# 0xC0000054/pdn-jpegxl

Hardware: AMD Instinct MI355X
Metric: megapixels/sec decode (4K lossy VarDCT) (higher is better)
Workload: dtype f32

## Files before the change

### pdn_jpegxl_amd/csrc/decoder.cc

```cpp
#include <hip/hip_runtime.h>
#include <algorithm>
#include <atomic>
#include <cmath>
#include <cstdarg>
#include <cstdio>
#include <cstdlib>
#include <cstring>
#include <memory>
#include <mutex>
#include <string>
#include <thread>
#include <vector>
#include "../../include/jxlfiletypeio.h"
#include "entropy_plan.h"
#include "host_parse.h"
#include "icc.h"
#include "kernels.h"

namespace jxlhip {

struct HipError : std::runtime_error {
  explicit HipError(const std::string& m) : std::runtime_error(m) {}
};
#define HIP_OK(expr)                                                                                      \
// ... 78 lines not shown
  hipStream_t own_stream = nullptr;
  float* d_basis_all = nullptr;
  float* d_basis_small = nullptr;
  float* d_basis_mfma = nullptr;
  float* d_llf_scale = nullptr;
  uint16_t* d_natural[kNumOrders] = {};
  U32x2* d_scan[kNumQuantTables] = {};
  float* d_dq[kNumQuantTables] = {};
  uint32_t dq_n[kNumQuantTables] = {};
  struct Tap { std::vector<uint8_t> qcoef[3], xyb_idct[3], xyb_filtered[3], noise_rnd[3], noise[3]; };
  struct Slot {
    uint8_t* d_ws = nullptr; size_t ws_cap = 0;
    uint8_t* d_blob = nullptr; size_t blob_cap = 0;
    uint8_t* h_blob = nullptr; size_t h_blob_cap = 0;
    uint32_t* h_status = nullptr; size_t h_status_cap = 0;
    int n = 0;
    std::vector<ParsedFrame> frames;
    int nfiles = 0;
    std::vector<int> file_of;
    std::vector<ParsedFrame> files;
    std::vector<DevImage> imgs;
    std::vector<int> parse_status;
    std::vector<std::string> parse_msg;
    std::vector<size_t> status_off;
    DevImage* d_imgs = nullptr;
    bool pending = false;
    hipEvent_t lf_done = nullptr, hf_done = nullptr, done = nullptr, uploaded = nullptr;
    std::vector<Tap> taps;
    std::vector<std::string> stage_names;
    std::vector<int> stage_chain;
    std::vector<hipEvent_t> events;
    std::vector<float> stage_ms;
  };
  static constexpr int kSlots = 3;
  static constexpr int kPixelChunk = 32;
  Slot slots[kSlots];
  int cur = 0, last = 0;
  Slot* active = &slots[0];
  hipStream_t stream_lf = nullptr;
  hipStream_t stream_hf = nullptr;
  hipStream_t last_stream = nullptr;
  std::vector<std::string> total_names;
  std::vector<double> total_ms;
  int total_batches = 0;
  std::string sticky_error;
  int sticky_status = 0;
  uint8_t* li_dev = nullptr; uint8_t* li_host = nullptr; size_t li_cap = 0;
  void EnsureLoadImageBuffers(size_t bytes);
  int lane_stride_override = 0;
  int hf_stride_override = 0;
  bool debug_taps = false;
  int band_first_row = 0, band_rows = 0;
  bool no_stream_pairs = false;
  bool no_lf_pipeline = false;
  bool no_direct = false, mod_lanes64 = false;
  bool overlap = true;
  int downscale = 1;

  explicit JxlHipDecoder(int dev);
  ~JxlHipDecoder();
  void EnsureWs(size_t bytes);
  void EnsureBlob(size_t bytes);
  void Mark(const char* name, hipStream_t s, int chain);
  void WaitSlot(Slot& S);
  Slot& Last() { return slots[last]; }
  void Decode(int32_t n_, const uint8_t* const* host_data, const size_t* sizes, const uint8_t* const* dev_data,
              uint8_t* const* dev_out, hipStream_t stream, bool sync, DecoderStatus* statuses, ErrorInfo* err);
  DecoderStatus Finish(DecoderStatus* statuses, ErrorInfo* err);
  void CopyPlaneTap(int stage);
  void PrepassSingle(ParsedFrame& f, const uint8_t* dev_file);
  EntropyPlanOptions PlanOptions() const;
};

JxlHipDecoder::JxlHipDecoder(int dev) {
  if (dev < 0) HIP_OK(hipGetDevice(&dev));
  device = dev;
  HIP_OK(hipSetDevice(device));
  int entropy_cus = 0, pixel_cus = 0;
  if (const char* e = Knob("JXLHIP_ENTROPY_CUS")) entropy_cus = std::min(256, std::max(0, atoi(e)));
  if (const char* e = Knob("JXLHIP_PIXEL_CUS")) pixel_cus = std::min(256, std::max(0, atoi(e)));
  auto masked_stream = [](hipStream_t* s, int first, int count) {
    uint32_t mask[8] = {0, 0, 0, 0, 0, 0, 0, 0};
    for (int i = first; i < first + count; i++) mask[i >> 5] |= 1u << (i & 31);
    HIP_OK(hipExtStreamCreateWithCUMask(s, 8, mask));
  };
  if (pixel_cus) masked_stream(&own_stream, 256 - pixel_cus, pixel_cus);
  else HIP_OK(hipStreamCreateWithFlags(&own_stream, hipStreamNonBlocking));
  int prio_least = 0, prio_greatest = 0;
  (void)hipDeviceGetStreamPriorityRange(&prio_least, &prio_greatest);
  const int prio = Knob("JXLHIP_NO_PRIORITY") ? prio_least : prio_greatest;
  if (entropy_cus) {
    masked_stream(&stream_lf, 0, entropy_cus);
    masked_stream(&stream_hf, 0, entropy_cus);
  } else {
    HIP_OK(hipStreamCreateWithPriority(&stream_lf, hipStreamNonBlocking, prio));
    HIP_OK(hipStreamCreateWithPriority(&stream_hf, hipStreamNonBlocking, prio));
  }
  for (auto& S : slots) {
    HIP_OK(hipEventCreateWithFlags(&S.lf_done, hipEventDisableTiming));
    HIP_OK(hipEventCreateWithFlags(&S.hf_done, hipEventDisableTiming));
    HIP_OK(hipEventCreateWithFlags(&S.done, hipEventDisableTiming));
    HIP_OK(hipEventCreateWithFlags(&S.uploaded, hipEventDisableTiming));
  }
  if (const char* e = Knob("JXLHIP_NO_OVERLAP")) overlap = atoi(e) == 0;
  const StaticTables& st = GetStaticTables();
  std::vector<float> all;
// ... 978 lines not shown
  if (s_lf != s_hf) {
    HIP_OK(hipEventRecord(S.lf_done, s_lf));
    HIP_OK(hipStreamWaitEvent(s_hf, S.lf_done, 0));
  }
#ifdef JXLHIP_EXPERIMENTS
  if (const char* e = Knob("JXLHIP_INTERFERE")) {
    int kind = 0, wgs = 1, lds_kb = 64; float ms = 100.f;
    if (sscanf(e, "%d,%d,%d,%f", &kind, &wgs, &lds_kb, &ms) >= 1 && kind >= 1 && kind <= 6 && wgs >= 1 && wgs <= 16 && lds_kb >= 1 && lds_kb <= 160 && ms > 0 && ms < 2000) {
      static hipStream_t xs = nullptr;
      static float* xbuf = nullptr;
      const size_t xbytes = (size_t)512 << 20;
      if (!xs) { HIP_OK(hipStreamCreateWithFlags(&xs, hipStreamNonBlocking)); HIP_OK(hipMalloc(&xbuf, xbytes)); }
      if (s_lf != s_hf) HIP_OK(hipStreamWaitEvent(xs, S.lf_done, 0));
      LaunchInterference(kind, wgs, lds_kb, ms, xbuf, xbytes, xs);
    }
  }
#endif
  Mark("hf_start", s_hf, 1);
  if (!(skip_stages & 2) && (!ds || npass_t))
  LaunchHfDecode(d_imgs, (const SectionTask*)(d_blob + off_pass_tasks), npass_t, plan.hf_waves * 64, plan.lane_stride, plan.hf.Bytes(), plan.lds_hf_lanes, s_hf);
  if (!ds || npass_t) Mark("hf_decode", s_hf, 1);
  if (any_alpha && !(skip_stages & 4))
    LaunchAlphaAns(d_imgs, (const SectionTask*)(d_blob + off_alpha_tasks), nalpha_t, plan.alpha_stride, plan.alpha.Bytes(), plan.direct_alpha, plan.lean_mod, s_hf);
  if (!ds || any_alpha) Mark("alpha_ans", s_hf, 1);
  if (debug_taps && !ds) {
    taps.assign(n, Tap());
    LaunchExpandCoefficients(d_imgs, n, true, max_tiles, stream);
    HIP_OK(hipStreamSynchronize(stream));
    CopyPlaneTap(0);
  }
  const bool finish_on_hf = s_hf == stream || debug_taps || !Knob("JXLHIP_ALPHA_FINISH_ON_PIX");
  if (finish_on_hf) {
    if (any_alpha && !(skip_stages & 4)) LaunchAlphaFinish(d_imgs, n, max_groups, s_hf);
    if (!ds || any_alpha) Mark("alpha_finish", s_hf, 1);
  }
  if (s_hf != stream) {
    HIP_OK(hipEventRecord(S.hf_done, s_hf));
    HIP_OK(hipStreamWaitEvent(stream, S.hf_done, 0));
  }
  Mark("main_start", stream, 2);
  if (!finish_on_hf) {
    if (any_alpha && !(skip_stages & 4)) LaunchAlphaFinish(d_imgs, n, max_groups, stream);
    Mark("alpha_finish", stream, 2);
  }
  hipStream_t s_pix = pix_on_hf ? s_hf : stream;
  if (ds && any_vardct) {
    if (any_alpha) LaunchAlphaReduce(d_imgs, n, max_ds_cells, s_pix);
    LaunchLfOutput(d_imgs, n, max_ds_cells, s_pix);
    Mark("lf_output", s_pix, 2);
  }
  for (int c0 = 0; c0 < (ds ? 0 : n); c0 += pixel_chunk) {
    const int cnt = std::min(pixel_chunk, n - c0);
    if (!(skip_stages & 8))
    LaunchReconTiles(d_imgs + c0, cnt, max_tiles, d_basis_all, d_basis_small, d_llf_scale, d_basis_mfma, s_pix);
    Mark("reconstruct", s_pix, 2);
    LaunchExpandCoefficients(d_imgs + c0, cnt, false, max_tiles, s_pix);
    LaunchGenericReconstruct(d_imgs + c0, cnt, d_basis_all, d_basis_small, d_llf_scale, s_pix);
    Mark("reconstruct_generic", s_pix, 2);
    if (debug_taps) { HIP_OK(hipStreamSynchronize(s_pix)); CopyPlaneTap(1); }
    if (any_noise && !(early_noise && c0 == 0)) { LaunchNoise(d_imgs + c0, cnt, max_groups, max_w, max_h, s_pix); Mark("noise", s_pix, 2); }
    if (!(skip_stages & 16))
    LaunchFilterTiles(d_imgs + c0, cnt, max_w, max_h, stage_mask, any_unfiltered, any_fused, any_fused2, s_pix);
    Mark("filters+output", s_pix, 2);
  }
  if (s_pix != stream) {
    HIP_OK(hipEventRecord(S.hf_done, s_pix));
    HIP_OK(hipStreamWaitEvent(stream, S.hf_done, 0));
  }
  if (nmod_t) {
    if (s_lf != stream) { HIP_OK(hipEventRecord(S.lf_done, s_lf)); HIP_OK(hipStreamWaitEvent(stream, S.lf_done, 0)); }
    LaunchModularAns(d_imgs, n, (const SectionTask*)(d_blob + off_mod_tasks), nmod_t, plan.mod.Bytes(), plan.max_mod_groups,
                     plan.max_mod_coded, plan.mod_lanes, plan.mod_rb, plan.mod_wp_lds, plan.direct_mod, stream);
    for (auto& op : mod_ops) {
      if (op.kind == 3) LaunchModularPalette(op.a, op.b, op.out, op.nout, op.type, op.rw, op.rh, op.status, stream);
      else LaunchModularOp(op.kind, op.a, op.b, op.c, op.aw, op.ah, op.rw, op.rh, op.type, stream);
    }
    LaunchModularOut(d_imgs, n, max_mod_pixels, stream);
    if (ds) LaunchBoxReduce(d_imgs, n, max_ds_cells, stream);
    Mark("modular", stream, 2);
  }
  if (!patch_tiles.empty()) {
    LaunchPatches((const PatchFrame*)(d_blob + off_patch_frames), (const PatchTile*)(d_blob + off_patch_tiles), (int)patch_tiles.size(),
                  (const int32_t*)(d_blob + off_patch_list), (const PatchPos*)(d_blob + off_patch_pos), (const PatchRef*)(d_blob + off_patch_refs),
                  stream);
    Mark("patches", stream, 2);
  }
  if (!comps.empty()) {
    LaunchCompose((const ComposeImage*)(d_blob + off_comp_imgs), (const ComposeFrame*)(d_blob + off_comp_frames), (int)comps.size(), max_segments, stream);
    Mark("compose", stream, 2);
  }
  for (int i = 0; i < n; i++)
    if (parse_status[i] == DecoderStatus_Ok && frames[i].orientation != 1 && !ds) {
      const ParsedFrame& f = frames[i];
      LaunchOrient(imgs[i].out, dev_out[i], (int)f.xsize, (int)f.ysize, (f.ncolor + (f.black_index >= 0 ? 1 : 0) + (f.alpha_index >= 0 ? 1 : 0)) * (int)OutBytesPerSample(f),
                   (int)f.orientation, stream);
    }
  LaunchStatusToHost((const uint32_t*)(d_ws + z_status_base), h_status, n * 16, stream);
  HIP_OK(hipEventRecord(S.done, stream));
  HIP_OK(hipGetLastError());
  last_stream = stream;
  S.pending = true;
  last = cur;
  cur = (cur + 1) % kSlots;
  (void)max_padded;
  if (sync) {
    DecoderStatus st = Finish(statuses, err);
    (void)st;
// ... 205 lines not shown
    info->num_channels = f.ncolor + (f.black_index >= 0 ? 1 : 0) + info->has_alpha;
    info->bytes_per_sample = (int32_t)OutBytesPerSample(f);
    info->reserved = f.exp_bits ? 1 : 0;
    info->xsize_blocks = f.w8; info->ysize_blocks = f.h8;
    info->num_groups = f.ng; info->num_lf_groups = f.nlf;
    info->epf_iters = f.epf_iters; info->gaborish = f.gab;
    info->codestream_bytes = f.cs_size;
    return DecoderStatus_Ok;
  } catch (const ParseError& e) {
    SetErr(err, "%s", e.what());
    return e.status;
  } catch (const std::exception& e) {
    SetErr(err, "%s", e.what());
    return DecoderStatus_DecodeError;
  }
}

DecoderStatus jxlhip_decode_batch(JxlHipDecoder* dec, int32_t n, const uint8_t* const* host_data, const size_t* sizes,
                                  const uint8_t* const* dev_data, uint8_t* const* dev_out, void* stream, int32_t synchronize,
                                  DecoderStatus* statuses, ErrorInfo* err) {
  if (!dec || !host_data || !sizes || !dev_out || n <= 0) return DecoderStatus_NullParameter;
  try {
    dec->Decode(n, host_data, sizes, dev_data, dev_out, (hipStream_t)stream, synchronize != 0, statuses, err);
    if (statuses) for (int i = 0; i < n; i++) if (statuses[i] != DecoderStatus_Ok) return statuses[i];
    return DecoderStatus_Ok;
  } catch (const std::bad_alloc&) {
    return DecoderStatus_OutOfMemory;
  } catch (const std::exception& e) {
    SetErr(err, "%s", e.what());
    return DecoderStatus_DecodeError;
  }
}

DecoderStatus jxlhip_finish(JxlHipDecoder* dec, DecoderStatus* statuses, ErrorInfo* err) {
  if (!dec) return DecoderStatus_NullParameter;
  try {
    return dec->Finish(statuses, err);
  } catch (const std::exception& e) {
    SetErr(err, "%s", e.what());
    return DecoderStatus_DecodeError;
  }
}

int32_t jxlhip_set_option(JxlHipDecoder* dec, const char* name, int32_t value) {
  if (!dec || !name) return 0;
  if (!strcmp(name, "debug_taps")) { dec->debug_taps = value != 0; return 1; }
  if (!strcmp(name, "query_pixel_chunk")) return JxlHipDecoder::kPixelChunk;
  if (!strcmp(name, "lane_stride")) { if (value != 0 && !PowerOfTwoUpTo64(value)) return 0; dec->lane_stride_override = value; return 1; }
  if (!strcmp(name, "band_first_row")) { if (value < 0) return 0; dec->band_first_row = value; return 1; }
  if (!strcmp(name, "band_rows")) { if (value < 0) return 0; dec->band_rows = value; return 1; }
  if (!strcmp(name, "no_direct")) { dec->no_direct = value != 0; return 1; }
  if (!strcmp(name, "no_stream_pairs")) { dec->no_stream_pairs = value != 0; return 1; }
  if (!strcmp(name, "no_lf_pipeline")) { dec->no_lf_pipeline = value != 0; return 1; }
  if (!strcmp(name, "mod_lanes64")) { dec->mod_lanes64 = value != 0; return 1; }
  if (!strcmp(name, "overlap")) { dec->overlap = value != 0; return 1; }
  if (!strcmp(name, "downscale")) { if (value != 1 && value != 8) return 0; dec->downscale = value; return 1; }
  return 0;
}

size_t jxlhip_read_plane(JxlHipDecoder* dec, int32_t index, const char* name, int32_t channel, void* dst, size_t capacity) {
  if (!dec || !name) return 0;
  JxlHipDecoder::Slot& S = dec->Last();
  if (index < 0 || index >= S.n || S.pending) return 0;
  if (S.parse_status[index] != DecoderStatus_Ok) return 0;
  const DevImage& d = S.imgs[index];
  std::string nm(name);
  const size_t cells = (size_t)d.w8 * d.h8, pix = (size_t)d.wp * d.hp;
  const void* src = nullptr;
  size_t bytes = 0;
  bool host = false;
  const int c = std::min(2, std::max(0, channel));
  if (nm == "lf") { src = d.lf_final[c]; bytes = cells * 4; }
  else if (nm == "lf_quant") { src = d.lfq[c]; bytes = cells * 4; }
  else if (nm == "cellinfo") { src = d.cellinfo; bytes = cells * 4; }
  else if (nm == "raw_quant") { src = d.rawq; bytes = cells * 2; }
  else if (nm == "sharpness") { src = d.sharp; bytes = cells; }
  else if (nm == "ytox") { src = d.ytox; bytes = (size_t)d.wt * d.ht; }
  else if (nm == "ytob") { src = d.ytob; bytes = (size_t)d.wt * d.ht; }
  else if (nm == "alpha") { src = d.alpha; bytes = (size_t)d.w * d.h; }
  else if (nm == "inv_sigma") { src = d.inv_sigma; bytes = cells * 4; }
  else if (dec->debug_taps && (size_t)index < S.taps.size()) {
    host = true;
    if (nm == "qcoef") { src = S.taps[index].qcoef[c].data(); bytes = S.taps[index].qcoef[c].size(); }
    else if (nm == "xyb_idct") { src = S.taps[index].xyb_idct[c].data(); bytes = S.taps[index].xyb_idct[c].size(); }
    else if (nm == "xyb_filtered") { src = S.taps[index].xyb_filtered[c].data(); bytes = S.taps[index].xyb_filtered[c].size(); }
    else if (nm == "noise_rnd") { src = S.taps[index].noise_rnd[c].data(); bytes = S.taps[index].noise_rnd[c].size(); }
    else if (nm == "noise") { src = S.taps[index].noise[c].data(); bytes = S.taps[index].noise[c].size(); }
  }
  (void)pix;
  if (!src || !bytes) return 0;
  if (dst && capacity) {
    size_t nb = std::min(bytes, capacity);
    if (host) memcpy(dst, src, nb);
    else if (hipMemcpy(dst, src, nb, hipMemcpyDeviceToHost) != hipSuccess) return 0;
  }
  return bytes;
}

int32_t jxlhip_stage_times(JxlHipDecoder* dec, const char** names, float* ms, int32_t capacity) {
  if (!dec) return 0;
  JxlHipDecoder::Slot& S = dec->Last();
  int32_t k = 0;
  for (size_t i = 1; i < S.stage_names.size() && i < S.stage_ms.size() && k < capacity; i++) {
    if (S.stage_ms[i] < 0.f) continue;
    if (names) names[k] = S.stage_names[i].c_str();
    if (ms) ms[k] = S.stage_ms[i];
// ... 210 lines not shown
```

### pdn_jpegxl_amd/csrc/kernels.h

```cpp
#pragma once
#include <hip/hip_runtime.h>
#include "dev_types.h"

namespace jxlhip {

void LaunchLfAns(const DevImage* imgs, const SectionTask* tasks, int ntasks, int slots, size_t lds_bytes, int scalar_rows, bool lean, hipStream_t s);
void LaunchLfFinish(const DevImage* imgs, const SectionTask* tasks, int ntasks, bool pipeline, hipStream_t s);
void LaunchHfBlockList(const DevImage* imgs, int nimg, int max_groups, hipStream_t s);
void LaunchHfDecode(const DevImage* imgs, const SectionTask* tasks, int nwg, int threads, int lane_stride, size_t lds_bytes, size_t lane_bytes,
                    hipStream_t s);
void LaunchAlphaAns(const DevImage* imgs, const SectionTask* tasks, int nwg, int lane_stride, size_t lds_bytes, int scalar_rows, bool lean, hipStream_t s);
void LaunchAlphaFinish(const DevImage* imgs, int nimg, int max_groups, hipStream_t s);
void LaunchModularAns(const DevImage* imgs, int nimg, const SectionTask* tasks, int ntasks, size_t lds_bytes, int max_sections, int max_coded,
                      int lanes, int rb_width, int wp_lds, int scalar_rows, hipStream_t s);
void LaunchModularOp(int kind, int32_t* a, int32_t* b, int32_t* c, int aw, int ah, int rw, int rh, int type, hipStream_t s);
void LaunchModularPalette(const int32_t* palette, const int32_t* index, int32_t* const* out, int nout, int nb_colors, int w, int h, uint32_t* status,
                          hipStream_t s);
void LaunchModularOut(const DevImage* imgs, int nimg, size_t max_pixels, hipStream_t s);
void LaunchOrient(const uint8_t* src, uint8_t* dst, int w, int h, int px_bytes, int orientation, hipStream_t s);
void LaunchLfPixelStages(const DevImage* imgs, int nimg, size_t max_cells, hipStream_t s);
void LaunchExpandCoefficients(const DevImage* imgs, int nimg, bool all_tiles, int max_tiles, hipStream_t s);
void LaunchGenericReconstruct(const DevImage* imgs, int nimg, const float* basis_all, const float* basis_small,
                              const float* llf_scale, hipStream_t s);
void LaunchReconTiles(const DevImage* imgs, int nimg, int max_tiles, const float* basis_all, const float* basis_small,
                      const float* llf_scale, const float* basis_mfma, hipStream_t s);
void LaunchFilterTiles(const DevImage* imgs, int nimg, int max_w, int max_h, int stage_mask, bool any_unfiltered,
                       int any_fused, int any_fused2, hipStream_t s);

void LaunchLfOutput(const DevImage* imgs, int nimg, size_t max_cells, hipStream_t s);
void LaunchAlphaReduce(const DevImage* imgs, int nimg, size_t max_cells, hipStream_t s);
void LaunchBoxReduce(const DevImage* imgs, int nimg, size_t max_cells, hipStream_t s);

void LaunchNoise(const DevImage* imgs, int nimg, int max_groups, int max_w, int max_h, hipStream_t s);

void LaunchCompose(const ComposeImage* imgs, const ComposeFrame* frames, int nimg, int max_segments, hipStream_t s);
void LaunchPatches(const PatchFrame* frames, const PatchTile* tiles, int ntiles, const int32_t* list, const PatchPos* pos, const PatchRef* refs,
                   hipStream_t s);

void LaunchStatusToHost(const uint32_t* src, uint32_t* dst_pinned, int nwords, hipStream_t s);
#ifdef JXLHIP_EXPERIMENTS
void LaunchInterference(int kind, int wg_per_cu, int lds_kb, float ms, float* scratch, size_t scratch_bytes, hipStream_t s);
#endif

}
```

### pdn_jpegxl_amd/csrc/tile_kernels.hip

```cpp
#include <hip/hip_runtime.h>
#include <cstdlib>
#include "dev_types.h"
#include "dev_util.h"
#include "kernels.h"

namespace jxlhip {

#ifndef JXLHIP_PRIO_PIXEL
#define JXLHIP_PRIO_PIXEL 0
#endif
#if JXLHIP_PRIO_PIXEL
#define JXL_PIXEL_PRIO() __builtin_amdgcn_s_setprio(JXLHIP_PRIO_PIXEL)
#else
#define JXL_PIXEL_PRIO() ((void)0)
#endif

namespace {

constexpr int kTS = 64;
constexpr int kLP = 65;

__device__ const uint8_t t_quant_table[kNumStrategies] = {0, 1, 2, 3, 4, 5, 6, 6, 7, 7, 8, 8, 9, 9, 10, 10, 10, 10, 11, 12, 12, 13, 14, 14, 15, 16, 16};

__device__ __forceinline__ bool Special(uint32_t s) { return (s >= 1 && s <= 3) || (s >= 12 && s <= 17); }
typedef float __attribute__((ext_vector_type(4))) F4;
template <int N>
__device__ __forceinline__ F4 MfmaChain(const float* pa, int sa, const float* pb, int sb) {
  float a[N / 4], b[N / 4];
#pragma unroll
  for (int k = 0; k < N / 4; k++) { a[k] = pa[k * sa]; b[k] = pb[k * sb]; }
  F4 acc = {0.f, 0.f, 0.f, 0.f};
#pragma unroll
  for (int k = 0; k < N / 4; k++) acc = __builtin_amdgcn_mfma_f32_16x16x4f32(a[k], b[k], acc, 0, 0, 0);
  return acc;
}
template <bool kTableIsA>
__device__ __forceinline__ F4 MfmaChain32L(const float4* t_lo, const float4* t_hi, int pair, const float* po, int so) {
  const float4 v0 = t_lo[pair], v1 = t_hi[pair];
  const float t[8] = {v0.x, v0.y, v0.z, v0.w, v1.x, v1.y, v1.z, v1.w};
  float o[8];
#pragma unroll
  for (int k = 0; k < 8; k++) o[k] = po[k * so];
  F4 acc = {0.f, 0.f, 0.f, 0.f};
#pragma unroll
  for (int k = 0; k < 8; k++)
    acc = kTableIsA ? __builtin_amdgcn_mfma_f32_16x16x4f32(t[k], o[k], acc, 0, 0, 0) : __builtin_amdgcn_mfma_f32_16x16x4f32(o[k], t[k], acc, 0, 0, 0);
  return acc;
}
template <bool kTableIsA>
__device__ __forceinline__ F4 MfmaChain64L(const float4* t64, int pair, const float* po, int so) {
  float t[16], o[16];
#pragma unroll
  for (int j = 0; j < 4; j++) {
    const float4 v = t64[j * 256 + pair];
    t[4 * j] = v.x; t[4 * j + 1] = v.y; t[4 * j + 2] = v.z; t[4 * j + 3] = v.w;
  }
#pragma unroll
  for (int k = 0; k < 16; k++) o[k] = po[k * so];
  F4 acc = {0.f, 0.f, 0.f, 0.f};
#pragma unroll
  for (int k = 0; k < 16; k++)
    acc = kTableIsA ? __builtin_amdgcn_mfma_f32_16x16x4f32(t[k], o[k], acc, 0, 0, 0) : __builtin_amdgcn_mfma_f32_16x16x4f32(o[k], t[k], acc, 0, 0, 0);
  return acc;
}
__device__ __forceinline__ bool MfmaRows(uint32_t tl, uint32_t tr) {
  return (tl >> 31) && (tr >> 31) && ((tl >> 21) & 7) >= 1 && ((tl >> 21) & 7) == ((tr >> 21) & 7) && ((tl >> 13) & 31) == ((tr >> 13) & 31);
}
__device__ __forceinline__ bool MfmaCols(uint32_t tl, uint32_t bl) {
  return (tl >> 31) && (bl >> 31) && ((tl >> 18) & 7) >= 1 && ((tl >> 18) & 7) == ((bl >> 18) & 7) && ((tl >> 8) & 31) == ((bl >> 8) & 31);
}

__device__ __forceinline__ float SrgbOetfT(float v) {
  const float lin = 12.92f * v;
  const float cur = 1.055f * __builtin_amdgcn_exp2f(__builtin_amdgcn_logf(v) * (1.0f / 2.4f)) - 0.055f;
  return v <= 0.0031308f ? lin : cur;
}
__device__ __forceinline__ float SrgbOetf255T(float v) {
  const float lin = (12.92f * 255.0f) * v;
  const float cur = (1.055f * 255.0f) * __builtin_amdgcn_exp2f(__builtin_amdgcn_logf(v) * (1.0f / 2.4f)) - (0.055f * 255.0f);
  return v <= 0.0031308f ? lin : cur;
}
__device__ __forceinline__ float PowT(float a, float e) { return __builtin_amdgcn_exp2f(__builtin_amdgcn_logf(a) * e); }
__device__ __forceinline__ float EncodeTransferT(int kind, float v, float pq_scale, const float* lut = nullptr) {
  if (kind == 0) return v;
  if (kind == 5) {
    const float t = __builtin_sqrtf(fminf(fmaxf(v, 0.f), 1.f)) * 4095.0f;
    const int i = min((int)t, 4094);
    return lut[i] + (lut[i + 1] - lut[i]) * (t - (float)i);
  }
  const float a = fabsf(v);
  float r;
  if (kind == 1) r = a <= 0.0031308f ? 12.92f * a : 1.055f * PowT(a, 1.0f / 2.4f) - 0.055f;
  else if (kind == 2) r = a < 0.018f ? 4.5f * a : 1.099f * PowT(a, 0.45f) - 0.099f;
  else {
    const float xp = a > 0.f ? PowT(a * pq_scale, 0.1593017578125f) : 0.f;
    r = a > 0.f ? PowT((0.8359375f + 18.8515625f * xp) / (1.0f + 18.6875f * xp), 78.84375f) : 0.f;
  }
  return copysignf(r, v);
}
__device__ __forceinline__ uint8_t ToU8T(float v) {
  v = fminf(fmaxf(v * 255.0f, 0.f), 255.0f);
  return (uint8_t)(v + 0.5f);
}

__device__ __forceinline__ uint32_t LoadAlpha(const DevImage& im, size_t i) {
  return im.out_bits == 8 ? (uint32_t)im.alpha[i] : (im.out_bits == 16 ? (uint32_t)((const uint16_t*)im.alpha)[i] : ((const uint32_t*)im.alpha)[i]);
}
template <typename Position>
__device__ __forceinline__ void WritePixelAt(const DevImage& im, Position position, float X, float Y, float B, uint32_t a) {
  const float gr = Y + X - im.opsin_bias_cbrt[0], gg = Y - X - im.opsin_bias_cbrt[1], gb = B - im.opsin_bias_cbrt[2];
  const float mr = gr * gr * gr + im.opsin_bias[0], mg = gg * gg * gg + im.opsin_bias[1], mb = gb * gb * gb + im.opsin_bias[2];
  float r = im.opsin_inv[0] * mr + im.opsin_inv[1] * mg + im.opsin_inv[2] * mb;
  float g = im.opsin_inv[3] * mr + im.opsin_inv[4] * mg + im.opsin_inv[5] * mb;
  float bl = im.opsin_inv[6] * mr + im.opsin_inv[7] * mg + im.opsin_inv[8] * mb;
  if (im.to_srgb == 1 && !im.out_float) {
    r = SrgbOetfT(r); g = SrgbOetfT(g); bl = SrgbOetfT(bl);
// ... 63 lines not shown
  float bl = im.opsin_inv[6] * mr + im.opsin_inv[7] * mg + im.opsin_inv[8] * mb;
  if (im.to_srgb) { r = SrgbOetf255T(r); g = SrgbOetf255T(g); bl = SrgbOetf255T(bl); }
  else { r *= 255.0f; g *= 255.0f; bl *= 255.0f; }
  uint32_t px = a << 24;
  px = __builtin_amdgcn_cvt_pk_u8_f32(r, 0, px);
  px = __builtin_amdgcn_cvt_pk_u8_f32(g, 1, px);
  px = __builtin_amdgcn_cvt_pk_u8_f32(bl, 2, px);
  return px;
}
__device__ __noinline__ void WritePixelGeneral(const DevImage& im, int x, int y, float X, float Y, float B, uint32_t a) {
  if (im.has_noise) {
    AddNoise(im, x, y, X, Y, B);
    if (im.out_bits == 8 && im.to_srgb <= 1 && !im.unpremultiply && im.final_stage == 5 &&
        (im.noise_pairs_twin || (im.nch_out == 4 && (x | 3) < im.w))) {
      const uint32_t px = PixelToRgba8(im, X, Y, B, a);
      uint8_t* out = im.out + ((size_t)(y - im.band_y0) * im.w + x) * im.nch_out;
      if (im.nch_out == 4) *(uint32_t*)out = px;
      else if (im.nch_out == 3) { out[0] = (uint8_t)px; out[1] = (uint8_t)(px >> 8); out[2] = (uint8_t)(px >> 16); }
      else { out[0] = (uint8_t)(px >> 8); if (im.nch_out == 2) out[1] = (uint8_t)(px >> 24); }
      return;
    }
  }
  WritePixelA(im, x, y, X, Y, B, a);
}
__device__ __forceinline__ void WritePixel(const DevImage& im, int x, int y, float X, float Y, float B) {
  const uint32_t a = im.has_alpha ? LoadAlpha(im, (size_t)y * im.w + x) : 0u;
  if (im.has_noise) { WritePixelGeneral(im, x, y, X, Y, B, a); return; }
  WritePixelA(im, x, y, X, Y, B, a);
}

}

#define JXL_IDCT_STEP(Bp, v0, v1)                                                                  \
  {                                                                                                \
    const float4 b0 = *(const float4*)(Bp);                                                        \
    const float4 b1 = *(const float4*)((Bp) + 4);                                                  \
    a0[0] += v0 * b0.x; a0[1] += v0 * b0.y; a0[2] += v0 * b0.z; a0[3] += v0 * b0.w;                \
    a0[4] += v0 * b1.x; a0[5] += v0 * b1.y; a0[6] += v0 * b1.z; a0[7] += v0 * b1.w;                \
    a1[0] += v1 * b0.x; a1[1] += v1 * b0.y; a1[2] += v1 * b0.z; a1[3] += v1 * b0.w;                \
    a1[4] += v1 * b1.x; a1[5] += v1 * b1.y; a1[6] += v1 * b1.z; a1[7] += v1 * b1.w;                \
  }

__device__ __forceinline__ float DequantBias(int32_t v, float qb, float qb3) {
  if (v == 0) return 0.f;
  if (v == 1) return qb;
  if (v == -1) return -qb;
  const float f = (float)v;
  return f - qb3 * __builtin_amdgcn_rcpf(f);
}
typedef int __attribute__((ext_vector_type(4))) I4v;

constexpr int kTileF = kTS * kLP;

__global__ __launch_bounds__(768, 6) void recon_tile_kernel(const DevImage* __restrict__ imgs, const float* basis_all, const float* basis_small,
                                                             const float* llf_scale, const float* basis_mfma) {
  JXL_PIXEL_PRIO();
  extern __shared__ __align__(16) uint8_t smem_raw[];
  float* cfc3 = (float*)smem_raw;
  float* B816 = cfc3 + 3 * kTileF;
  float* cscale = B816 + 320;
  uint32_t* ci = (uint32_t*)(cscale + 64);
  uint32_t* cmeta = ci + 64;
  uint32_t* cnq = cmeta + 64;
  uint32_t* cpre = cnq + 64;
  uint32_t* cstart = cpre + 3 * 64;
  uint32_t* ctot = cstart + 3 * 64;
  const U32x2** csc = (const U32x2**)(ctot + 4);
  float4* t32_lo = (float4*)(csc + 64);
  float4* t32_hi = t32_lo + 128;
  float4* t64 = t32_hi + 128;
  const DevImage& im = imgs[blockIdx.y];
  const int tile = blockIdx.x;
  if (tile >= im.wt * im.ht) return;
  const int tid = threadIdx.x;
  const int tx = tile % im.wt, ty = tile / im.wt;
  if (ty < im.dec_gy0 * 4 || ty >= im.dec_gy1 * 4) return;
  const int wave = tid >> 6, lane = tid & 63, team = wave >> 2, tw = wave & 3;
  const int c = team == 0 ? 1 : (team == 1 ? 0 : 2);
  const int wp = im.wp, hp = im.hp;
  {
    float4* z = (float4*)cfc3;
    for (int i = tid; i < 3 * kTileF / 4; i += 768) z[i] = make_float4(0.f, 0.f, 0.f, 0.f);
  }
  int bad = 0, has64 = 0;
  if (tid < 64) {
    const int cx = tx * 8 + (tid & 7), cy = ty * 8 + (tid >> 3);
    const bool inside = cx < im.w8 && cy < im.h8;
    const size_t cell_g = (size_t)min(cy, im.h8 - 1) * im.w8 + min(cx, im.w8 - 1);
    const size_t ncells = (size_t)im.w8 * im.h8;
    const uint32_t info_g = im.cellinfo[cell_g];
    const uint32_t rq_g = im.rawq[cell_g];
    U32x2 blk[3];
    blk[0] = im.cblk[ncells + cell_g]; blk[1] = im.cblk[cell_g]; blk[2] = im.cblk[2 * ncells + cell_g];
    const uint32_t info = inside ? info_g : 0u;
    const uint32_t rqv = inside ? rq_g : 1u;
    const int ix = (info >> 8) & 31, iy = (info >> 13) & 31, lcx = (info >> 18) & 7, lcy = (info >> 21) & 7;
    if (inside) {
      if (!(info >> 31)) bad = 1;
      else {
        const int ox = (tid & 7) - ix, oy = (tid >> 3) - iy;
        bad = ox < 0 || oy < 0 || ox + (1 << lcx) > 8 || oy + (1 << lcy) > 8 || Special(info & 0xFF) ||
              (ox & ((1 << lcx) - 1)) != 0 || (oy & ((1 << lcy) - 1)) != 0;
      }
    }
    const bool valid = (info >> 31) && !bad;
    has64 = valid && (lcx == 3 || lcy == 3);
    {
      const uint64_t any = __ballot(has64);
      if (tid == 0) ctot[3] = any != 0;
    }
    const uint32_t q = t_quant_table[valid ? (info & 0xFF) : 0];
    const uint32_t rq_origin = (uint32_t)__shfl((int)rqv, valid ? tid - iy * 8 - ix : tid);
    const uint32_t lng = 3 + max(lcx, lcy);
    const bool transposed = lcy >= lcx;
    ci[tid] = info;
    cscale[tid] = im.inv_global_scale / (float)rq_origin;
    cmeta[tid] = lng | (transposed ? 16u : 0u);
    cnq[tid] = im.dq_n[q];
    csc[tid] = im.scan[q];
    const bool origin = valid && ix == 0 && iy == 0;
    uint32_t cnt[3], sum[3];
#pragma unroll
    for (int t = 0; t < 3; t++) {
      cnt[t] = origin ? blk[t].y : 0u;
      if (cnt[t] > 65536u || blk[t].x > kGroupEntriesCap - cnt[t]) cnt[t] = 0;
      sum[t] = cnt[t];
    }
#pragma unroll
    for (int d = 1; d < 64; d <<= 1) {
#pragma unroll
      for (int t = 0; t < 3; t++) {
        const uint32_t a = (uint32_t)__shfl_up((int)sum[t], d);
        if (tid >= d) sum[t] += a;
      }
    }
#pragma unroll
    for (int t = 0; t < 3; t++) {
      cpre[t * 64 + tid] = sum[t] - cnt[t];
      cstart[t * 64 + tid] = blk[t].x;
      if (tid == 63) ctot[t] = sum[t];
    }
  } else if (tid < 64 + 320) {
    B816[tid - 64] = basis_all[tid - 64];
  } else if (tid < 64 + 320 + 256) {
    const int i = tid - (64 + 320);
    const float4 v = ((const float4*)basis_mfma)[i];
    if (i & 1) t32_hi[i >> 1] = v; else t32_lo[i >> 1] = v;
  }
  if (im.num_passes > 1) bad = 1;
  if (__syncthreads_or(bad)) {
    if (tid == 0) im.tile_list[atomicAdd(&im.status[1], 1u)] = (uint32_t)tile;
    return;
  }
  if (ctot[3]) {
    for (int i = tid; i < 1024; i += 768) t64[(i & 3) * 256 + (i >> 2)] = ((const float4*)(basis_mfma + 1024))[i];
  }
  const float* const Bl = basis_all;
  float* const cfc = cfc3 + team * kTileF;
  if (tw == 0) {
    const int cxg = tx * 8 + (lane & 7), cyg = ty * 8 + (lane >> 3);
    const bool inside = cxg < im.w8 && cyg < im.h8;
    const float lf_g = im.lf_final[c][(size_t)min(cyg, im.h8 - 1) * im.w8 + min(cxg, im.w8 - 1)];
    const float lfv = inside ? lf_g : 0.f;
    const uint32_t info = ci[lane];
    const bool valid = info >> 31;
    const int ix = (info >> 8) & 31, iy = (info >> 13) & 31, lcx = (info >> 18) & 7, lcy = (info >> 21) & 7;
    const int cx = 1 << lcx, cy = 1 << lcy;
    const int ox = (lane & 7) - ix, oy = (lane >> 3) - iy;
    const float* Bx = basis_small + (cx * cx - 1) / 3 + ix * cx;
    const float* By = basis_small + (cy * cy - 1) / 3 + iy * cy;
    float bx[8], byv[8];
#pragma unroll
    for (int k = 0; k < 8; k++) { bx[k] = (valid && k < cx) ? Bx[k] : 0.f; byv[k] = (valid && k < cy) ? By[k] : 0.f; }
    const float sc = valid ? llf_scale[lcy * 32 + iy] * llf_scale[lcx * 32 + ix] / (float)(cx * cy) : 0.f;
    float row = 0.f;
#pragma unroll
    for (int k = 0; k < 8; k++) {
      const float v = __shfl(lfv, (lane - ix + k) & 63);
      if (valid && k < cx) row += v * bx[k];
    }
    float acc = 0.f;
#pragma unroll
    for (int k = 0; k < 8; k++) {
      const float v = __shfl(row, ((oy + k) * 8 + (lane & 7)) & 63);
      if (valid && k < cy) acc += v * byv[k];
    }
    if (valid) atomicAdd(&cfc[(oy * 8 + iy) * kLP + ox * 8 + ix], acc * sc);
  }
  {
    const size_t tile_cfl = (size_t)ty * im.wt + tx;
    const float cfl_x = im.base_x + (float)im.ytox[tile_cfl] * im.inv_color_factor;
    const float cfl_b = im.base_b + (float)im.ytob[tile_cfl] * im.inv_color_factor;
    const uint32_t* entries = im.centries + (size_t)((ty >> 2) * im.xg + (tx >> 2) - im.centries_g0) * kGroupEntriesCap;
    const uint32_t t0 = ctot[0], t01 = t0 + ctot[1], total = t01 + ctot[2];
    const float qb3 = im.qbias[3];
    for (uint32_t e = (uint32_t)tid; e < total; e += 768) {
      const uint32_t t = (e >= t0) + (e >= t01);
      const uint32_t el = e - (t == 0 ? 0u : (t == 1 ? t0 : t01));
      const uint32_t* pre = cpre + t * 64;
      uint32_t j = 0;
#pragma unroll
      for (int step = 32; step; step >>= 1) if (pre[j + step] <= el) j += step;
      const uint32_t ent = entries[cstart[t * 64 + j] + (el - pre[j])];
      const uint32_t k = ent & 0xFFFFu, nq = cnq[j];
      if (k >= nq) continue;
      const int chan = t == 0 ? 1 : (t == 1 ? 0 : 2);
      const U32x2 se = csc[j][(size_t)chan * nq + k];
      const uint32_t meta = cmeta[j];
      const uint32_t lng = meta & 15, p = se.x;
      const uint32_t r = p >> lng, cc = p & ((1u << lng) - 1);
      const uint32_t ky = (meta & 16) ? cc : r, kx = (meta & 16) ? r : cc;
      if (ky >= 64 || kx >= 64) continue;
      const int32_t v = (int32_t)ent >> 16;
      const float dm = t == 0 ? 1.0f : (t == 1 ? im.x_dm : im.b_dm);
      const float o = DequantBias(v, im.qbias[chan], qb3) * (cscale[j] * dm) * __uint_as_float(se.y);
      const uint32_t at = ((j >> 3) * 8 + ky) * kLP + (j & 7) * 8 + kx;
      atomicAdd(&cfc3[t * kTileF + at], o);
      if (t == 0) {
        if (cfl_x != 0.f) atomicAdd(&cfc3[kTileF + at], o * cfl_x);
        if (cfl_b != 0.f) atomicAdd(&cfc3[2 * kTileF + at], o * cfl_b);
      }
    }
  }
  __syncthreads();
  const int l16 = tid & 15, lq = lane >> 4;
  {
    F4 acc[4];
    bool m[4];
    const int x0 = tw * 16;
#pragma unroll
    for (int rb = 0; rb < 4; rb++) {
      const uint32_t inf = ci[rb * 16 + tw * 2];
      m[rb] = MfmaRows(inf, ci[rb * 16 + tw * 2 + 1]);
      if (m[rb]) {
        const int iy = (inf >> 13) & 31, lcy = (inf >> 21) & 7, R = 8 << lcy;
        const float* cp = cfc + ((rb * 2 - iy) * 8 + lq) * kLP + x0 + l16;
        if (R == 16) acc[rb] = MfmaChain<16>(B816 + 64 + lq * 16 + iy * 8 + l16, 64, cp, 4 * kLP);
        else if (R == 32) acc[rb] = MfmaChain32L<true>(t32_lo, t32_hi, (iy * 8 + l16) * 4 + lq, cp, 4 * kLP);
        else acc[rb] = MfmaChain64L<true>(t64, (iy * 8 + l16) * 4 + lq, cp, 4 * kLP);
      }
    }
    const int x = x0 + (lane & 7) * 2, cr = lane >> 3;
    const uint32_t info = ci[cr * 8 + (x >> 3)];
    const bool valu = (info >> 31) && !MfmaRows(ci[(cr >> 1) * 16 + (x >> 4) * 2], ci[(cr >> 1) * 16 + (x >> 4) * 2 + 1]);
    float a0[8] = {0, 0, 0, 0, 0, 0, 0, 0}, a1[8] = {0, 0, 0, 0, 0, 0, 0, 0};
    if (valu) {
      const int iy = (info >> 13) & 31, lcy = (info >> 21) & 7;
      const int R = 8 << lcy;
      const float* in = cfc + (cr - iy) * 8 * kLP + x;
      if (R == 8) {
#pragma unroll 2
        for (int k = 0; k < 8; k++) { const float v0 = in[k * kLP], v1 = in[k * kLP + 1]; JXL_IDCT_STEP(B816 + k * 8, v0, v1) }
      } else if (R == 16) {
        const float* B = B816 + 64 + iy * 8;
#pragma unroll 2
        for (int k = 0; k < 16; k++) { const float v0 = in[k * kLP], v1 = in[k * kLP + 1]; JXL_IDCT_STEP(B + k * 16, v0, v1) }
      } else {
        const float* B = Bl + (R * R - 64) / 3 + iy * 8;
        for (int k = 0; k < R; k++) { const float v0 = in[k * kLP], v1 = in[k * kLP + 1]; JXL_IDCT_STEP(B + k * R, v0, v1) }
      }
    }
    __builtin_amdgcn_fence(__ATOMIC_RELEASE, "wavefront");
    __builtin_amdgcn_wave_barrier();
#pragma unroll
    for (int rb = 0; rb < 4; rb++)
      if (m[rb]) {
        float* o = cfc + (rb * 16 + 4 * lq) * kLP + x0 + l16;
        o[0] = acc[rb].x; o[kLP] = acc[rb].y; o[2 * kLP] = acc[rb].z; o[3 * kLP] = acc[rb].w;
      }
    if (valu) {
#pragma unroll
      for (int j = 0; j < 8; j++) { cfc[(cr * 8 + j) * kLP + x] = a0[j]; cfc[(cr * 8 + j) * kLP + x + 1] = a1[j]; }
    }
  }
  __syncthreads();
  {
    F4 acc[4];
    bool m[4];
    const int y0 = tw * 16;
#pragma unroll
    for (int cs = 0; cs < 4; cs++) {
      const uint32_t inf = ci[tw * 16 + cs * 2];
      m[cs] = MfmaCols(inf, ci[tw * 16 + 8 + cs * 2]);
      if (m[cs]) {
        const int ix = (inf >> 8) & 31, lcx = (inf >> 18) & 7, C = 8 << lcx;
        const float* ap = cfc + (y0 + l16) * kLP + (cs * 2 - ix) * 8 + lq;
        if (C == 16) acc[cs] = MfmaChain<16>(ap, 4, B816 + 64 + lq * 16 + ix * 8 + l16, 64);
        else if (C == 32) acc[cs] = MfmaChain32L<false>(t32_lo, t32_hi, (ix * 8 + l16) * 4 + lq, ap, 4);
        else acc[cs] = MfmaChain64L<false>(t64, (ix * 8 + l16) * 4 + lq, ap, 4);
      }
    }
    const int y = y0 + (lane & 7) * 2, cc = lane >> 3;
    const uint32_t info = ci[(y >> 3) * 8 + cc];
    const bool valu = (info >> 31) && !MfmaCols(ci[(y >> 4) * 16 + (cc >> 1) * 2], ci[(y >> 4) * 16 + 8 + (cc >> 1) * 2]);
    float a0[8] = {0, 0, 0, 0, 0, 0, 0, 0}, a1[8] = {0, 0, 0, 0, 0, 0, 0, 0};
    if (valu) {
      const int ix = (info >> 8) & 31, lcx = (info >> 18) & 7;
      const int C = 8 << lcx;
      const float* in = cfc + y * kLP + (cc - ix) * 8;
      if (C == 8) {
#pragma unroll 2
        for (int k = 0; k < 8; k++) { const float v0 = in[k], v1 = in[k + kLP]; JXL_IDCT_STEP(B816 + k * 8, v0, v1) }
      } else if (C == 16) {
        const float* B = B816 + 64 + ix * 8;
#pragma unroll 2
        for (int k = 0; k < 16; k++) { const float v0 = in[k], v1 = in[k + kLP]; JXL_IDCT_STEP(B + k * 16, v0, v1) }
      } else {
        const float* B = Bl + (C * C - 64) / 3 + ix * 8;
        for (int k = 0; k < C; k++) { const float v0 = in[k], v1 = in[k + kLP]; JXL_IDCT_STEP(B + k * C, v0, v1) }
      }
    }
    __builtin_amdgcn_fence(__ATOMIC_RELEASE, "wavefront");
    __builtin_amdgcn_wave_barrier();
#pragma unroll
    for (int cs = 0; cs < 4; cs++)
      if (m[cs]) {
        float* o = cfc + (y0 + 4 * lq) * kLP + cs * 16 + l16;
        o[0] = acc[cs].x; o[kLP] = acc[cs].y; o[2 * kLP] = acc[cs].z; o[3 * kLP] = acc[cs].w;
      }
    if (valu) {
#pragma unroll
      for (int j = 0; j < 8; j++) { cfc[y * kLP + cc * 8 + j] = a0[j]; cfc[(y + 1) * kLP + cc * 8 + j] = a1[j]; }
    }
    __builtin_amdgcn_fence(__ATOMIC_ACQ_REL, "wavefront");
    __builtin_amdgcn_wave_barrier();
    float* dst = im.xyb[c];
    const int x4 = l16 * 4;
    const int gx = tx * kTS + x4;
#pragma unroll
    for (int it = 0; it < 4; it++) {
      const int yl = y0 + lq + 4 * it;
      const int gy = ty * kTS + yl;
      const float* r = cfc + yl * kLP + x4;
      const float4 o = make_float4(r[0], r[1], r[2], r[3]);
      if (gx < wp && gy < hp) *(float4*)(dst + (size_t)gy * wp + gx) = o;
    }
  }
}

template <int kStage>
__global__ __launch_bounds__(256) void filter_tile_kernel(const DevImage* __restrict__ imgs) {
  JXL_PIXEL_PRIO();
// ... 639 lines not shown
  }
}

__device__ __forceinline__ void LfOutputPixel(const DevImage& im, size_t i, float X, float Y, float B) {
  const int cx = (int)(i % (size_t)im.ds_w), cy = (int)(i / (size_t)im.ds_w);
  const size_t o = OrientedIndex(im.ds_orient, cx, cy, im.ds_w, im.ds_h);
  const uint32_t a = !im.has_alpha ? 0u : (im.out_bits == 8 ? (uint32_t)im.ds_alpha[i] : (im.out_bits == 16 ? (uint32_t)((const uint16_t*)im.ds_alpha)[i]
                                                                                                              : ((const uint32_t*)im.ds_alpha)[i]));
  if (PlainOutput(im)) {
    const uint32_t px = PixelToRgba8(im, X, Y, B, a);
    uint8_t* out = im.out + o * im.nch_out;
    if (im.nch_out == 4) *(uint32_t*)out = px;
    else if (im.nch_out == 3) { out[0] = (uint8_t)px; out[1] = (uint8_t)(px >> 8); out[2] = (uint8_t)(px >> 16); }
    else { out[0] = (uint8_t)(px >> 8); if (im.nch_out == 2) out[1] = (uint8_t)(px >> 24); }
    return;
  }
  WritePixelAt(im, [&] { return o; }, X, Y, B, a);
}
__global__ __launch_bounds__(256) void lf_output_kernel(const DevImage* __restrict__ imgs) {
  const DevImage& im = imgs[blockIdx.y];
  if (!im.ds || im.is_modular) return;
  const size_t n = (size_t)im.ds_w * im.ds_h;
  const float* __restrict__ pX = im.lf_final[0];
  const float* __restrict__ pY = im.lf_final[1];
  const float* __restrict__ pB = im.lf_final[2];
  const size_t gid = (size_t)blockIdx.x * blockDim.x + threadIdx.x, stride = (size_t)gridDim.x * blockDim.x;
  const bool quads = PlainOutput(im) && im.ds_orient == 1 && im.ncolor == 3 && ((uintptr_t)im.out & 15) == 0;
  if (!quads) {
    for (size_t i = gid; i < n; i += stride) LfOutputPixel(im, i, pX[i], pY[i], pB[i]);
    return;
  }
  const size_t nq = n >> 2;
  for (size_t q = gid; q < nq; q += stride) {
    const float4 X = ((const float4*)pX)[q], Y = ((const float4*)pY)[q], B = ((const float4*)pB)[q];
    const uint32_t a = im.has_alpha ? ((const uint32_t*)im.ds_alpha)[q] : 0u;
    const uint32_t p0 = PixelToRgba8(im, X.x, Y.x, B.x, a & 0xFF), p1 = PixelToRgba8(im, X.y, Y.y, B.y, (a >> 8) & 0xFF);
    const uint32_t p2 = PixelToRgba8(im, X.z, Y.z, B.z, (a >> 16) & 0xFF), p3 = PixelToRgba8(im, X.w, Y.w, B.w, a >> 24);
    if (im.nch_out == 4) ((uint4*)im.out)[q] = make_uint4(p0, p1, p2, p3);
    else ((uint3*)im.out)[q] = make_uint3((p0 & 0xFFFFFFu) | (p1 << 24), ((p1 >> 8) & 0xFFFFu) | (p2 << 16), ((p2 >> 16) & 0xFFu) | (p3 << 8));
  }
  if (blockIdx.x == 0 && threadIdx.x < (n & 3)) {
    const size_t i = 4 * nq + threadIdx.x;
    LfOutputPixel(im, i, pX[i], pY[i], pB[i]);
  }
}

void LaunchLfOutput(const DevImage* imgs, int nimg, size_t max_cells, hipStream_t s) {
  if (nimg <= 0) return;
  const size_t b = std::min<size_t>((max_cells + 255) / 256, 2048);
  hipLaunchKernelGGL(lf_output_kernel, dim3((unsigned)std::max<size_t>(1, b), nimg), dim3(256), 0, s, imgs);
}

void LaunchReconTiles(const DevImage* imgs, int nimg, int max_tiles, const float* basis_all, const float* basis_small,
                      const float* llf_scale, const float* basis_mfma, hipStream_t s) {
  const size_t lds = (size_t)(3 * kTileF + 320 + 64 * 4 + 64 * 6 + 4 + 128 + 1024 + 4096) * 4;
  static bool raised = false;
  if (!raised) { (void)hipFuncSetAttribute((const void*)recon_tile_kernel, hipFuncAttributeMaxDynamicSharedMemorySize, (int)lds); raised = true; }
  hipLaunchKernelGGL(recon_tile_kernel, dim3(max_tiles, nimg), dim3(768), lds, s, imgs, basis_all, basis_small, llf_scale, basis_mfma);
}

void LaunchFilterTiles(const DevImage* imgs, int nimg, int max_w, int max_h, int stage_mask, bool any_unfiltered,
                       int any_fused, int any_fused2, hipStream_t s) {
  const int tiles = ((max_w + 63) / 64) * ((max_h + 31) / 32);
  dim3 g(tiles, nimg);
  if (stage_mask & 1) hipLaunchKernelGGL(filter_tile_kernel<0>, g, dim3(256), 0, s, imgs);
  if (stage_mask & 2) hipLaunchKernelGGL(filter_tile_kernel<1>, g, dim3(256), 0, s, imgs);
  if (any_fused) {
    const int groups = ((max_w + kStripOut - 1) / kStripOut) * ((max_h + 2 + kSegRows - 1) / kSegRows);
    const int pair_groups = ((max_w + kPairOut - 1) / kPairOut) * ((max_h + 2 + kSegRows - 1) / kSegRows);
    if (any_fused & 1) hipLaunchKernelGGL(filter_stream_pairs_kernel, dim3((pair_groups + kGroupsPerWg - 1) / kGroupsPerWg, nimg), dim3(256), 0, s, imgs);
    if (any_fused & 2) hipLaunchKernelGGL(filter_stream_kernel, dim3((groups + kGroupsPerWg - 1) / kGroupsPerWg, nimg), dim3(256), 0, s, imgs);
    const int pair2_groups = ((max_w + kPair2Out - 1) / kPair2Out) * ((max_h + kSegRows - 1) / kSegRows);
    if (any_fused2 & 1) hipLaunchKernelGGL(filter_stream2_pairs_kernel, dim3((pair2_groups + kGroupsPerWg - 1) / kGroupsPerWg, nimg), dim3(256), 0, s, imgs);
    if (any_fused2 & 2) hipLaunchKernelGGL(filter_stream2_kernel, dim3((groups + kGroupsPerWg - 1) / kGroupsPerWg, nimg), dim3(256), 0, s, imgs);
  }
  if (stage_mask & 4) hipLaunchKernelGGL(filter_tile_kernel<2>, g, dim3(256), 0, s, imgs);
  if (stage_mask & 8) hipLaunchKernelGGL(filter_tile_kernel<3>, g, dim3(256), 0, s, imgs);
  if (any_unfiltered) {
    size_t work = (size_t)max_w * max_h;
    size_t b = std::min<size_t>((work + 255) / 256, 8192);
    hipLaunchKernelGGL(out_only_kernel, dim3((unsigned)b, nimg), dim3(256), 0, s, imgs);
  }
}

}
```

Measured before the change: 32040.

## Track nonzero coefficient bounds per block to shorten MFMA IDCT chains

During coefficient scatter, the kernel records per-block maximum nonzero row and column indices in shared memory using atomicMax. The MFMA row and column IDCT passes use these bounds to pick a shorter templated chain length, and skip row passes whose columns are all zero. This aims to cut matrix-multiply work on sparse high-frequency blocks in large transforms. In exchange it adds atomics during dequant, more template instantiations (raising code size and register pressure), a slightly larger LDS footprint, and a launch_bounds occupancy hint raised from 6 to 7.

```diff
diff --git a/pdn_jpegxl_amd/csrc/decoder.cc b/pdn_jpegxl_amd/csrc/decoder.cc
--- a/pdn_jpegxl_amd/csrc/decoder.cc
+++ b/pdn_jpegxl_amd/csrc/decoder.cc
@@ -154,6 +154,7 @@
   bool debug_taps = false;
   int band_first_row = 0, band_rows = 0;
   bool no_stream_pairs = false;
+  bool no_recon_bounds = false;
   bool no_lf_pipeline = false;
   bool no_direct = false, mod_lanes64 = false;
   bool overlap = true;
@@ -1238,7 +1239,7 @@
   for (int c0 = 0; c0 < (ds ? 0 : n); c0 += pixel_chunk) {
     const int cnt = std::min(pixel_chunk, n - c0);
     if (!(skip_stages & 8))
-    LaunchReconTiles(d_imgs + c0, cnt, max_tiles, d_basis_all, d_basis_small, d_llf_scale, d_basis_mfma, s_pix);
+    LaunchReconTiles(d_imgs + c0, cnt, max_tiles, d_basis_all, d_basis_small, d_llf_scale, d_basis_mfma, !no_recon_bounds, s_pix);
     Mark("reconstruct", s_pix, 2);
     LaunchExpandCoefficients(d_imgs + c0, cnt, false, max_tiles, s_pix);
     LaunchGenericReconstruct(d_imgs + c0, cnt, d_basis_all, d_basis_small, d_llf_scale, s_pix);
@@ -1550,6 +1551,7 @@
   if (!strcmp(name, "no_direct")) { dec->no_direct = value != 0; return 1; }
   if (!strcmp(name, "no_stream_pairs")) { dec->no_stream_pairs = value != 0; return 1; }
   if (!strcmp(name, "no_lf_pipeline")) { dec->no_lf_pipeline = value != 0; return 1; }
+  if (!strcmp(name, "no_recon_bounds")) { dec->no_recon_bounds = value != 0; return 1; }
   if (!strcmp(name, "mod_lanes64")) { dec->mod_lanes64 = value != 0; return 1; }
   if (!strcmp(name, "overlap")) { dec->overlap = value != 0; return 1; }
   if (!strcmp(name, "downscale")) { if (value != 1 && value != 8) return 0; dec->downscale = value; return 1; }
diff --git a/pdn_jpegxl_amd/csrc/kernels.h b/pdn_jpegxl_amd/csrc/kernels.h
--- a/pdn_jpegxl_amd/csrc/kernels.h
+++ b/pdn_jpegxl_amd/csrc/kernels.h
@@ -23,7 +23,7 @@
 void LaunchGenericReconstruct(const DevImage* imgs, int nimg, const float* basis_all, const float* basis_small,
                               const float* llf_scale, hipStream_t s);
 void LaunchReconTiles(const DevImage* imgs, int nimg, int max_tiles, const float* basis_all, const float* basis_small,
-                      const float* llf_scale, const float* basis_mfma, hipStream_t s);
+                      const float* llf_scale, const float* basis_mfma, bool use_bounds, hipStream_t s);
 void LaunchFilterTiles(const DevImage* imgs, int nimg, int max_w, int max_h, int stage_mask, bool any_unfiltered,
                        int any_fused, int any_fused2, hipStream_t s);
 
diff --git a/pdn_jpegxl_amd/csrc/tile_kernels.hip b/pdn_jpegxl_amd/csrc/tile_kernels.hip
--- a/pdn_jpegxl_amd/csrc/tile_kernels.hip
+++ b/pdn_jpegxl_amd/csrc/tile_kernels.hip
@@ -34,34 +34,44 @@
   for (int k = 0; k < N / 4; k++) acc = __builtin_amdgcn_mfma_f32_16x16x4f32(a[k], b[k], acc, 0, 0, 0);
   return acc;
 }
-template <bool kTableIsA>
-__device__ __forceinline__ F4 MfmaChain32L(const float4* t_lo, const float4* t_hi, int pair, const float* po, int so) {
-  const float4 v0 = t_lo[pair], v1 = t_hi[pair];
-  const float t[8] = {v0.x, v0.y, v0.z, v0.w, v1.x, v1.y, v1.z, v1.w};
-  float o[8];
-#pragma unroll
-  for (int k = 0; k < 8; k++) o[k] = po[k * so];
+template <int KS, bool kTableIsA>
+__device__ __forceinline__ F4 MfmaChainL(const float4* tq, int qs, int pair, const float* po, int so) {
+  constexpr int Q = (KS + 3) / 4;
+  float t[4 * Q], o[KS];
+#pragma unroll
+  for (int j = 0; j < Q; j++) {
+    const float4 v = tq[j * qs + pair];
+    t[4 * j] = v.x; t[4 * j + 1] = v.y; t[4 * j + 2] = v.z; t[4 * j + 3] = v.w;
+  }
+#pragma unroll
+  for (int k = 0; k < KS; k++) o[k] = po[k * so];
   F4 acc = {0.f, 0.f, 0.f, 0.f};
 #pragma unroll
-  for (int k = 0; k < 8; k++)
+  for (int k = 0; k < KS; k++)
     acc = kTableIsA ? __builtin_amdgcn_mfma_f32_16x16x4f32(t[k], o[k], acc, 0, 0, 0) : __builtin_amdgcn_mfma_f32_16x16x4f32(o[k], t[k], acc, 0, 0, 0);
   return acc;
 }
+__device__ __forceinline__ F4 MfmaChain16T(const float* pa, int sa, const float* pb, int sb, int ks) {
+  if (ks <= 1) return MfmaChain<4>(pa, sa, pb, sb);
+  if (ks <= 2) return MfmaChain<8>(pa, sa, pb, sb);
+  if (ks <= 3) return MfmaChain<12>(pa, sa, pb, sb);
+  return MfmaChain<16>(pa, sa, pb, sb);
+}
 template <bool kTableIsA>
-__device__ __forceinline__ F4 MfmaChain64L(const float4* t64, int pair, const float* po, int so) {
-  float t[16], o[16];
-#pragma unroll
-  for (int j = 0; j < 4; j++) {
-    const float4 v = t64[j * 256 + pair];
-    t[4 * j] = v.x; t[4 * j + 1] = v.y; t[4 * j + 2] = v.z; t[4 * j + 3] = v.w;
-  }
-#pragma unroll
-  for (int k = 0; k < 16; k++) o[k] = po[k * so];
-  F4 acc = {0.f, 0.f, 0.f, 0.f};
-#pragma unroll
-  for (int k = 0; k < 16; k++)
-    acc = kTableIsA ? __builtin_amdgcn_mfma_f32_16x16x4f32(t[k], o[k], acc, 0, 0, 0) : __builtin_amdgcn_mfma_f32_16x16x4f32(o[k], t[k], acc, 0, 0, 0);
-  return acc;
+__device__ __forceinline__ F4 MfmaChain32T(const float4* t32, int pair, const float* po, int so, int ks) {
+  if (ks <= 1) return MfmaChainL<1, kTableIsA>(t32, 128, pair, po, so);
+  if (ks <= 2) return MfmaChainL<2, kTableIsA>(t32, 128, pair, po, so);
+  if (ks <= 4) return MfmaChainL<4, kTableIsA>(t32, 128, pair, po, so);
+  if (ks <= 6) return MfmaChainL<6, kTableIsA>(t32, 128, pair, po, so);
+  return MfmaChainL<8, kTableIsA>(t32, 128, pair, po, so);
+}
+template <bool kTableIsA>
+__device__ __forceinline__ F4 MfmaChain64T(const float4* t64, int pair, const float* po, int so, int ks) {
+  if (ks <= 2) return MfmaChainL<2, kTableIsA>(t64, 256, pair, po, so);
+  if (ks <= 4) return MfmaChainL<4, kTableIsA>(t64, 256, pair, po, so);
+  if (ks <= 8) return MfmaChainL<8, kTableIsA>(t64, 256, pair, po, so);
+  if (ks <= 12) return MfmaChainL<12, kTableIsA>(t64, 256, pair, po, so);
+  return MfmaChainL<16, kTableIsA>(t64, 256, pair, po, so);
 }
 __device__ __forceinline__ bool MfmaRows(uint32_t tl, uint32_t tr) {
   return (tl >> 31) && (tr >> 31) && ((tl >> 21) & 7) >= 1 && ((tl >> 21) & 7) == ((tr >> 21) & 7) && ((tl >> 13) & 31) == ((tr >> 13) & 31);
@@ -231,8 +241,8 @@
 
 constexpr int kTileF = kTS * kLP;
 
-__global__ __launch_bounds__(768, 6) void recon_tile_kernel(const DevImage* __restrict__ imgs, const float* basis_all, const float* basis_small,
-                                                             const float* llf_scale, const float* basis_mfma) {
+__global__ __launch_bounds__(768, 7) void recon_tile_kernel(const DevImage* __restrict__ imgs, const float* basis_all, const float* basis_small,
+                                                             const float* llf_scale, const float* basis_mfma, int use_bounds) {
   JXL_PIXEL_PRIO();
   extern __shared__ __align__(16) uint8_t smem_raw[];
   float* cfc3 = (float*)smem_raw;
@@ -248,6 +258,8 @@
   float4* t32_lo = (float4*)(csc + 64);
   float4* t32_hi = t32_lo + 128;
   float4* t64 = t32_hi + 128;
+  uint32_t* brow = (uint32_t*)(t64 + 1024);
+  uint32_t* bcol = brow + 64;
   const DevImage& im = imgs[blockIdx.y];
   const int tile = blockIdx.x;
   if (tile >= im.wt * im.ht) return;
@@ -297,6 +309,8 @@
     cmeta[tid] = lng | (transposed ? 16u : 0u);
     cnq[tid] = im.dq_n[q];
     csc[tid] = im.scan[q];
+    brow[tid] = 1u << lcy;
+    bcol[tid] = 1u << lcx;
     const bool origin = valid && ix == 0 && iy == 0;
     uint32_t cnt[3], sum[3];
 #pragma unroll
@@ -395,6 +409,8 @@
       const float o = DequantBias(v, im.qbias[chan], qb3) * (cscale[j] * dm) * __uint_as_float(se.y);
       const uint32_t at = ((j >> 3) * 8 + ky) * kLP + (j & 7) * 8 + kx;
       atomicAdd(&cfc3[t * kTileF + at], o);
+      if (ky >= __atomic_load_n(&brow[j], __ATOMIC_RELAXED)) atomicMax(&brow[j], ky + 1);
+      if (kx >= __atomic_load_n(&bcol[j], __ATOMIC_RELAXED)) atomicMax(&bcol[j], kx + 1);
       if (t == 0) {
         if (cfl_x != 0.f) atomicAdd(&cfc3[kTileF + at], o * cfl_x);
         if (cfl_b != 0.f) atomicAdd(&cfc3[2 * kTileF + at], o * cfl_b);
@@ -412,11 +428,21 @@
       const uint32_t inf = ci[rb * 16 + tw * 2];
       m[rb] = MfmaRows(inf, ci[rb * 16 + tw * 2 + 1]);
       if (m[rb]) {
+        const uint32_t inr = ci[rb * 16 + tw * 2 + 1];
         const int iy = (inf >> 13) & 31, lcy = (inf >> 21) & 7, R = 8 << lcy;
-        const float* cp = cfc + ((rb * 2 - iy) * 8 + lq) * kLP + x0 + l16;
-        if (R == 16) acc[rb] = MfmaChain<16>(B816 + 64 + lq * 16 + iy * 8 + l16, 64, cp, 4 * kLP);
-        else if (R == 32) acc[rb] = MfmaChain32L<true>(t32_lo, t32_hi, (iy * 8 + l16) * 4 + lq, cp, 4 * kLP);
-        else acc[rb] = MfmaChain64L<true>(t64, (iy * 8 + l16) * 4 + lq, cp, 4 * kLP);
+        const int ixl = (inf >> 8) & 31, ixr = (inr >> 8) & 31;
+        const int ol = (rb * 2 - iy) * 8 + tw * 2 - ixl, orr = (rb * 2 - iy) * 8 + tw * 2 + 1 - ixr;
+        int ks = R >> 2;
+        if (use_bounds) {
+          ks = __builtin_amdgcn_readfirstlane((int)(max(brow[ol], brow[orr]) + 3) >> 2);
+          m[rb] = __builtin_amdgcn_readfirstlane(ixl * 8 < (int)bcol[ol] || ixr * 8 < (int)bcol[orr]);
+        }
+        if (m[rb]) {
+          const float* cp = cfc + ((rb * 2 - iy) * 8 + lq) * kLP + x0 + l16;
+          if (R == 16) acc[rb] = MfmaChain16T(B816 + 64 + lq * 16 + iy * 8 + l16, 64, cp, 4 * kLP, ks);
+          else if (R == 32) acc[rb] = MfmaChain32T<true>(t32_lo, (iy * 8 + l16) * 4 + lq, cp, 4 * kLP, ks);
+          else acc[rb] = MfmaChain64T<true>(t64, (iy * 8 + l16) * 4 + lq, cp, 4 * kLP, ks);
+        }
       }
     }
     const int x = x0 + (lane & 7) * 2, cr = lane >> 3;
@@ -462,11 +488,15 @@
       const uint32_t inf = ci[tw * 16 + cs * 2];
       m[cs] = MfmaCols(inf, ci[tw * 16 + 8 + cs * 2]);
       if (m[cs]) {
+        const uint32_t inb = ci[tw * 16 + 8 + cs * 2];
         const int ix = (inf >> 8) & 31, lcx = (inf >> 18) & 7, C = 8 << lcx;
+        const int ot = (tw * 2 - (int)((inf >> 13) & 31)) * 8 + cs * 2 - ix, ob = (tw * 2 + 1 - (int)((inb >> 13) & 31)) * 8 + cs * 2 - ix;
+        int ks = C >> 2;
+        if (use_bounds) ks = __builtin_amdgcn_readfirstlane((int)(max(bcol[ot], bcol[ob]) + 3) >> 2);
         const float* ap = cfc + (y0 + l16) * kLP + (cs * 2 - ix) * 8 + lq;
-        if (C == 16) acc[cs] = MfmaChain<16>(ap, 4, B816 + 64 + lq * 16 + ix * 8 + l16, 64);
-        else if (C == 32) acc[cs] = MfmaChain32L<false>(t32_lo, t32_hi, (ix * 8 + l16) * 4 + lq, ap, 4);
-        else acc[cs] = MfmaChain64L<false>(t64, (ix * 8 + l16) * 4 + lq, ap, 4);
+        if (C == 16) acc[cs] = MfmaChain16T(ap, 4, B816 + 64 + lq * 16 + ix * 8 + l16, 64, ks);
+        else if (C == 32) acc[cs] = MfmaChain32T<false>(t32_lo, (ix * 8 + l16) * 4 + lq, ap, 4, ks);
+        else acc[cs] = MfmaChain64T<false>(t64, (ix * 8 + l16) * 4 + lq, ap, 4, ks);
       }
     }
     const int y = y0 + (lane & 7) * 2, cc = lane >> 3;
@@ -1212,11 +1242,11 @@
 }
 
 void LaunchReconTiles(const DevImage* imgs, int nimg, int max_tiles, const float* basis_all, const float* basis_small,
-                      const float* llf_scale, const float* basis_mfma, hipStream_t s) {
-  const size_t lds = (size_t)(3 * kTileF + 320 + 64 * 4 + 64 * 6 + 4 + 128 + 1024 + 4096) * 4;
+                      const float* llf_scale, const float* basis_mfma, bool use_bounds, hipStream_t s) {
+  const size_t lds = (size_t)(3 * kTileF + 320 + 64 * 4 + 64 * 6 + 4 + 128 + 1024 + 4096 + 2 * 64) * 4;
   static bool raised = false;
   if (!raised) { (void)hipFuncSetAttribute((const void*)recon_tile_kernel, hipFuncAttributeMaxDynamicSharedMemorySize, (int)lds); raised = true; }
-  hipLaunchKernelGGL(recon_tile_kernel, dim3(max_tiles, nimg), dim3(768), lds, s, imgs, basis_all, basis_small, llf_scale, basis_mfma);
+  hipLaunchKernelGGL(recon_tile_kernel, dim3(max_tiles, nimg), dim3(768), lds, s, imgs, basis_all, basis_small, llf_scale, basis_mfma, use_bounds ? 1 : 0);
 }
 
 void LaunchFilterTiles(const DevImage* imgs, int nimg, int max_w, int max_h, int stage_mask, bool any_unfiltered,
```

Result: no change. 32570, median of 3 (+1.6%).
